# google/layered-scene-inference

Hardware: AMD Instinct MI355X
Metric: rendered views/sec (BxLxHxW splat+warp) (higher is better)
Workload: dtype f32; 1 GPU; cfg3: 4-layer LDI 256x768, batch 32 per GPU (32 total), trg_downsampling 0.5, kitti cameras, compose_layers, smooth disparities; launch=graph, input_sets_rotated=3, parallelism=batch-sharded replicas x1 (no collective)

## Files before the change

include/lsi_hip.h:

```cpp
#ifndef LSI_HIP_H_
#define LSI_HIP_H_

#include <stddef.h>
#include <stdint.h>

#ifdef __cplusplus
extern "C" {
#endif

#define LSI_VERSION 100

#define LSI_OK 0
#define LSI_EINVAL -1
#define LSI_ENULL -2
#define LSI_EWORKSPACE -3
#define LSI_ELAUNCH -4
#define LSI_EUNSUPPORTED -5

#define LSI_COMPOSE 1u
#define LSI_WANT_DISP 2u
#define LSI_HAS_MASK 4u
#define LSI_WS_KEEP 8u
#define LSI_DETERMINISTIC 16u

#define LSI_PACKED_RGBD 32u
#define LSI_GRAD_M 64u

#define LSI_PATH_AUTO 0
#define LSI_PATH_ATOMIC 1
#define LSI_PATH_ROWBAND 2
#define LSI_PATH_STREAM 3

#define LSI_PATH_TILE 4

typedef void* lsi_stream_t;

typedef struct LsiStreamAdapt {
  int32_t state;
  int32_t pending;
  uint32_t seq;
  uint32_t calls;
  uint32_t* ctr_dev;
  volatile uint32_t* ctr_host;
} LsiStreamAdapt;

typedef struct LsiSplatDesc {
  int32_t L, B, H, W, Ht, Wt;
  int64_t tex_sl, tex_sb, tex_sy, tex_sx, tex_sc;
  int64_t disp_sl, disp_sb, disp_sy, disp_sx;
  int64_t mask_sl, mask_sb, mask_sy, mask_sx;
  float trg_downsampling;
  float max_disp;
  float zbuf_scale;
  float bg_wt;
  uint32_t flags;
  int32_t path;
  int32_t tune_rows, tune_threads, tune_window, reserved;
  LsiStreamAdapt* adapt;
} LsiSplatDesc;

int lsi_version(void);

const char* lsi_strerror(int code);

float lsi_bg_weight(double bg_layer_disp, double max_disp, double zbuf_scale);

int lsi_rowband_ok(const LsiSplatDesc* desc, const float* M_host);

int lsi_stream_ok(const LsiSplatDesc* desc, const float* M_host);

size_t lsi_splat_workspace_bytes(const LsiSplatDesc* desc);

int lsi_splat_fwd(const LsiSplatDesc* desc, const float* tex, const float* disp,
                  const float* mask, const float* M, float* out_img,
                  float* out_wts, float* out_disp, void* workspace,
                  size_t workspace_bytes, lsi_stream_t stream);

size_t lsi_splat_bwd_workspace_bytes(const LsiSplatDesc* desc);

int lsi_splat_bwd(const LsiSplatDesc* desc, const float* tex, const float* disp,
                  const float* mask, const float* M, const float* out_img,
                  const float* out_wts, const float* g_img, const float* g_wts,
                  float* g_tex, float* g_disp_in, float* g_mask,
                  void* workspace, size_t workspace_bytes, lsi_stream_t stream);

int lsi_splat_bwd_m(const LsiSplatDesc* desc, const float* tex,
                    const float* disp, const float* mask, const float* M,
                    const float* out_img, const float* out_wts,
                    const float* g_img, const float* g_wts, float* g_tex,
                    float* g_disp_in, float* g_mask, float* g_M, void* workspace,
                    size_t workspace_bytes, lsi_stream_t stream);

size_t lsi_splat_bwd_disp_workspace_bytes(const LsiSplatDesc* desc);

int lsi_splat_bwd_disp(const LsiSplatDesc* desc, const float* tex,
                       const float* disp, const float* mask, const float* M,
                       const float* out_img, const float* out_wts,
                       const float* out_disp, const float* g_img,
                       const float* g_wts, const float* g_disp_out,
                       float* g_tex, float* g_disp_in, float* g_mask,
                       float* g_M, void* workspace, size_t workspace_bytes,
                       lsi_stream_t stream);

int lsi_splat_fwd_both(const LsiSplatDesc* desc, const float* tex,
                       const float* disp, const float* mask, const float* M,
                       float* out_img, float* out_wts, float* out_img_c,
                       float* out_wts_c, void* workspace,
                       size_t workspace_bytes, lsi_stream_t stream);

int lsi_splat_bwd_both(const LsiSplatDesc* desc, const float* tex,
                       const float* disp, const float* mask, const float* M,
                       const float* out_img, const float* out_wts,
                       const float* out_img_c, const float* out_wts_c,
                       const float* g_img, const float* g_wts,
                       const float* g_img_c, const float* g_wts_c, float* g_tex,
                       float* g_disp_in, float* g_mask, void* workspace,
                       size_t workspace_bytes, lsi_stream_t stream);

int lsi_splat_bwd_both_m(const LsiSplatDesc* desc, const float* tex,
                         const float* disp, const float* mask, const float* M,
                         const float* out_img, const float* out_wts,
                         const float* out_img_c, const float* out_wts_c,
                         const float* g_img, const float* g_wts,
                         const float* g_img_c, const float* g_wts_c,
                         float* g_tex, float* g_disp_in, float* g_mask,
                         float* g_M, void* workspace, size_t workspace_bytes,
                         lsi_stream_t stream);

int lsi_project_indices(const LsiSplatDesc* desc, const float* disp,
                        const float* mask, const float* M, int32_t* idx4,
                        float* upd4, lsi_stream_t stream);

int lsi_splat_generic(int32_t B, int32_t Hs, int32_t Ws, int32_t C, int32_t Ht,
                      int32_t Wt, const float* src, const float* coords,
                      float* out, lsi_stream_t stream);

int lsi_splat_generic_bwd(int32_t B, int32_t Hs, int32_t Ws, int32_t C,
                          int32_t Ht, int32_t Wt, const float* src,
                          const float* coords, const float* g_out, float* g_src,
                          float* g_coords, lsi_stream_t stream);

int lsi_projection_matrices(int32_t B, const float* k_s, const float* k_t,
                            const float* rot, const float* t, int32_t inverse,
                            float* M);

int lsi_scatter_add(int32_t B, int64_t P, int64_t N, const int32_t* idx,
                    const float* upd, float* out, lsi_stream_t stream);

int lsi_bilinear_fwd(int32_t B, int32_t Hs, int32_t Ws, int32_t C, int32_t Ht,
                     int32_t Wt, const float* imgs, const float* coords,
                     float* out, lsi_stream_t stream);

int lsi_bilinear_taps(int32_t B, int32_t Hs, int32_t Ws, int32_t C, int32_t Ht,
                      int32_t Wt, const float* imgs, const float* coords,
                      float* taps, float* wts, lsi_stream_t stream);
int lsi_bilinear_taps_bwd(int32_t B, int32_t Hs, int32_t Ws, int32_t C, int32_t Ht,
                          int32_t Wt, const float* coords, const float* g_taps,
                          const float* g_wts, float* g_imgs, float* g_coords,
                          lsi_stream_t stream);

int lsi_bilinear_bwd(int32_t B, int32_t Hs, int32_t Ws, int32_t C, int32_t Ht,
// ... 445 lines not shown
```

layered-scene-inference_amd/csrc/lsi_splat_bwd_stream.hip:

```cpp
#include <hip/hip_runtime.h>
#include <math.h>
#include <stdint.h>
#include <stdlib.h>

#include <type_traits>

#include "../../include/lsi_hip.h"
#include "lsi_common.h"
#include "lsi_splat_internal.h"

#pragma clang fp contract(off)

using namespace lsi;

namespace {

constexpr int BS_WPE = 2;
constexpr int BS_FENCE = 1;
constexpr int BS_T = 512;
constexpr int BS_NW = BS_T / 64;
constexpr int BS_SEG = 256;

struct BSCanvas {
  const float* img;
  const float* wts;
  const float* g_img;
  const float* g_wts;
};

struct BSArgs {
  const float* tex;
  const float* disp;
  const float* M;
  const float* mask;
  float* g_mask;
  int mask_sb, mask_sl, mask_sy;
  BSCanvas ci, cc;
  int vec4;
  float* g_tex;
  float* g_disp;
  int nt;
  int B, H, W, Ht, Wt, L, nseg;
  int tex_sb, tex_sl, tex_sy, disp_sb, disp_sl, disp_sy;
  float s, max_disp, zscale, zA, zB;
  int compose;
  int remap;
  int RS;
  int GR;
  float* gm_part;
  const float2* gd;
};

struct BSIn { float4 d4, t0, t1, t2, mk; };

__device__ __forceinline__ float4 bs_pre(float i0, float i1, float i2, float w,
                                         float g0, float g1, float g2, float gw) {
  const float inv = 1.0f / safe_den(w);
  return make_float4(g0 * inv, g1 * inv, g2 * inv,
                     gw - (g0 * i0 + g1 * i1 + g2 * i2) * inv);
}
__device__ __forceinline__ float4 bs_cell(const BSCanvas& c, size_t o) {
  return bs_pre(c.img[3 * o], c.img[3 * o + 1], c.img[3 * o + 2], c.wts[o],
                c.g_img[3 * o], c.g_img[3 * o + 1], c.g_img[3 * o + 2],
                c.g_wts ? c.g_wts[o] : 0.0f);
}
__device__ __forceinline__ float4 bs_G(const BSArgs& a, size_t oi, size_t oc) {
  float4 g = make_float4(0.f, 0.f, 0.f, 0.f);
  if (a.cc.g_img) g = bs_cell(a.cc, oc);
  if (a.ci.g_img) {
    const float4 h = bs_cell(a.ci, oi);
    g.x += h.x; g.y += h.y; g.z += h.z; g.w += h.w;
  }
  return g;
}
__device__ __forceinline__ void bs_cell4(const BSCanvas& c, size_t o, float4 (&g)[4],
                                         bool add) {
  const float4 ia = *reinterpret_cast<const float4*>(c.img + 3 * o);
  const float4 ib = *reinterpret_cast<const float4*>(c.img + 3 * o + 4);
  const float4 ic = *reinterpret_cast<const float4*>(c.img + 3 * o + 8);
  const float4 w = *reinterpret_cast<const float4*>(c.wts + o);
  const float4 ga = *reinterpret_cast<const float4*>(c.g_img + 3 * o);
  const float4 gb = *reinterpret_cast<const float4*>(c.g_img + 3 * o + 4);
  const float4 gc = *reinterpret_cast<const float4*>(c.g_img + 3 * o + 8);
  float4 gw = make_float4(0.f, 0.f, 0.f, 0.f);
  if (c.g_wts) gw = *reinterpret_cast<const float4*>(c.g_wts + o);
  float4 h[4];
  h[0] = bs_pre(ia.x, ia.y, ia.z, w.x, ga.x, ga.y, ga.z, gw.x);
  h[1] = bs_pre(ia.w, ib.x, ib.y, w.y, ga.w, gb.x, gb.y, gw.y);
  h[2] = bs_pre(ib.z, ib.w, ic.x, w.z, gb.z, gb.w, gc.x, gw.z);
  h[3] = bs_pre(ic.y, ic.z, ic.w, w.w, gc.y, gc.z, gc.w, gw.w);
#pragma unroll
  for (int k = 0; k < 4; ++k) {
    if (add) { g[k].x += h[k].x; g[k].y += h[k].y; g[k].z += h[k].z; g[k].w += h[k].w; }
    else g[k] = h[k];
  }
}

template <bool PACK>
__device__ __forceinline__ void bs_load(BSIn& o, const float* pd, const float* pt) {
  if (PACK) {
    o.d4 = *reinterpret_cast<const float4*>(pt);
    o.t0 = *reinterpret_cast<const float4*>(pt + 4);
    o.t1 = *reinterpret_cast<const float4*>(pt + 8);
    o.t2 = *reinterpret_cast<const float4*>(pt + 12);
  } else {
    o.d4 = *reinterpret_cast<const float4*>(pd);
    o.t0 = *reinterpret_cast<const float4*>(pt);
    o.t1 = *reinterpret_cast<const float4*>(pt + 4);
    o.t2 = *reinterpret_cast<const float4*>(pt + 8);
  }
}

typedef float __attribute__((ext_vector_type(4))) bs_f4v;
typedef const __attribute__((address_space(3))) bs_f4v bs_lds_f4;

template <bool IN_LDS, bool PACK, bool MASK, bool GRAD_M, bool WANT_DISP>
__device__ __forceinline__ void bs_run(const BSArgs& a, const float (&m)[8],
                                       BSIn (&set)[2], const float4* gt,
                                       size_t obi, size_t obc, int b,
                                       int l_lo, int NL, int ys, int nitem,
                                       int glo, int wave, int lane,
                                       float (&acc)[16]) {
  const int Wt = a.Wt, nseg = a.nseg;
  const int half = (Wt + 1) >> 1;
  const float s = a.s;
  const float xmax = (float)Wt - 1.0f, ymax = (float)a.Ht - 1.0f;
  const float inv_md = div_rn(1.0f, a.max_disp);
  const float zs_md = a.zscale * inv_md;
  const float* const g_tex_in = a.tex + (long)b * a.tex_sb + (long)l_lo * a.tex_sl;
  const float* const g_disp_in = a.disp + (long)b * a.disp_sb + (long)l_lo * a.disp_sl;
  const int px_last = a.W - 4;
  const float* const g_mask_in =
      MASK ? a.mask + (long)b * a.mask_sb + (long)l_lo * a.mask_sl : nullptr;
  float* const o_mask =
      MASK ? a.g_mask + ((size_t)l_lo * a.B + b) * ((size_t)a.H * a.W) + 4 * lane : nullptr;
  float* const o_tex = a.g_tex + ((size_t)l_lo * a.B + b) * ((size_t)a.H * a.W) * 3 + 12 * lane;
  float* const o_disp = a.g_disp + ((size_t)l_lo * a.B + b) * ((size_t)a.H * a.W) + 4 * lane;
  const size_t lay_px = (size_t)a.B * a.H * a.W;
  bs_lds_f4* const gt3 = (bs_lds_f4*)gt;

  struct Pos { int r, sg, l; };
  auto advance = [&](Pos& p, int n) {
    p.l += n;
    while (p.l >= NL) { p.l -= NL; ++p.sg; }
    while (p.sg >= nseg) { p.sg -= nseg; ++p.r; }
  };
  auto load_item = [&](BSIn& o, const Pos& p, bool live) {
    const Pos q = live ? p : Pos{0, 0, 0};
    const int px = min(q.sg * BS_SEG + 4 * lane, px_last);
    bs_load<PACK>(o, g_disp_in + (long)q.l * a.disp_sl + (long)(ys + q.r) * a.disp_sy + px,
                  g_tex_in + (long)q.l * a.tex_sl + (long)(ys + q.r) * a.tex_sy + (PACK ? 4 : 3) * px);
    if (MASK)
      o.mk = *reinterpret_cast<const float4*>(
          g_mask_in + (long)q.l * a.mask_sl + (long)(ys + q.r) * a.mask_sy + px);
  };
  auto item = [&](const BSIn& in, const Pos& p) {
    const int y = ys + p.r, sg = p.sg, l = p.l;
    const float py = (float)y + 0.5f;
    const float q1 = mrow(m, 1, 0.5f, py, 0.0f);
    const float Y = q1 * s - 0.5f;
    const Axis ay = splat_axis(Y, ymax);
    const bool yok = finite_f(Y);
    const int r0 = yok ? (int)ay.c0s : glo, r1 = yok ? (int)ay.c1s : glo;
    const float pym01 = py * m[1];
    const float dvn[4] = {in.d4.x, in.d4.y, in.d4.z, in.d4.w};
    const float dvp[4] = {in.d4.w, in.t0.w, in.t1.w, in.t2.w};
    const float txn[12] = {in.t0.x, in.t0.y, in.t0.z, in.t0.w, in.t1.x, in.t1.y,
                           in.t1.z, in.t1.w, in.t2.x, in.t2.y, in.t2.z, in.t2.w};
    const float txp[12] = {in.d4.x, in.d4.y, in.d4.z, in.t0.x, in.t0.y, in.t0.z,
                           in.t1.x, in.t1.y, in.t1.z, in.t2.x, in.t2.y, in.t2.z};
    const float (&dv)[4] = PACK ? dvp : dvn;
    const float (&tx)[12] = PACK ? txp : txn;
    const float mkv[4] = {in.mk.x, in.mk.y, in.mk.z, in.mk.w};
    float ot[12], od[4], om[4];
#pragma unroll
    for (int i = 0; i < 4; ++i) {
      const float d = dv[i];
      const float t0 = tx[3 * i], t1 = tx[3 * i + 1], t2 = tx[3 * i + 2];
      const float px = (float)(sg * BS_SEG + 4 * lane + i) + 0.5f;
      const float q0 = ((px * m[0] + pym01) + m[2]) + d * m[3];
      const float X = q0 * s - 0.5f;
      const bool ok = yok && finite_f(X) && finite_f(d);
      const Axis ax = splat_axis(X, xmax);
      float w0 = clamp_small(ax.w0 * ay.w0), w1 = clamp_small(ax.w1 * ay.w0);
      float w2 = clamp_small(ax.w0 * ay.w1), w3 = clamp_small(ax.w1 * ay.w1);
      if (!ok) { w0 = 0.f; w1 = 0.f; w2 = 0.f; w3 = 0.f; }
      const int c0 = ok ? (int)ax.c0s : 0, c1 = ok ? (int)ax.c1s : 0;
      float4 g0, g1, g2, g3;
      if (IN_LDS) {
        bs_lds_f4* ra = gt3 + (r0 - glo) * Wt;
        bs_lds_f4* rb = gt3 + (r1 - glo) * Wt;
        const int s0 = (c0 >> 1) + (c0 & 1) * half, s1 = (c1 >> 1) + (c1 & 1) * half;
        const bs_f4v v0 = ra[s0], v1 = ra[s1], v2 = rb[s0], v3 = rb[s1];
        g0 = make_float4(v0.x, v0.y, v0.z, v0.w); g1 = make_float4(v1.x, v1.y, v1.z, v1.w);
        g2 = make_float4(v2.x, v2.y, v2.z, v2.w); g3 = make_float4(v3.x, v3.y, v3.z, v3.w);
      } else {
        const size_t ra = (size_t)r0 * Wt, rb = (size_t)r1 * Wt;
        g0 = bs_G(a, obi + ra + c0, obc + ra + c0);
        g1 = bs_G(a, obi + ra + c1, obc + ra + c1);
        g2 = bs_G(a, obi + rb + c0, obc + rb + c0);
        g3 = bs_G(a, obi + rb + c1, obc + rb + c1);
      }
      float gsd = 0.0f;
      if (WANT_DISP) {
        const float2* gdl = a.gd + ((size_t)(l_lo + l) * a.B + b) * ((size_t)a.Ht * Wt);
        const size_t ra = (size_t)r0 * Wt, rb = (size_t)r1 * Wt;
        const float2 e0 = gdl[ra + c0], e1 = gdl[ra + c1];
        const float2 e2 = gdl[rb + c0], e3 = gdl[rb + c1];
        const float dz = ok ? d : 0.0f;
        g0.w = g0.w + (e0.y + dz * e0.x); g1.w = g1.w + (e1.y + dz * e1.x);
        g2.w = g2.w + (e2.y + dz * e2.x); g3.w = g3.w + (e3.y + dz * e3.x);
        gsd = __fmaf_rn(w3, e3.x, __fmaf_rn(w2, e2.x, __fmaf_rn(w1, e1.x, w0 * e0.x)));
      }
      const float xn = d * inv_md;
      const float ez = __builtin_amdgcn_exp2f(
          __fmaf_rn(__builtin_amdgcn_fmed3f(d, 0.0f, a.max_disp), a.zA, a.zB));
      const float zw = xn > 0.0f ? ez : 0.0f;
      const float S0 = __fmaf_rn(t0, g0.x, __fmaf_rn(t1, g0.y, __fmaf_rn(t2, g0.z, g0.w)));
      const float S1 = __fmaf_rn(t0, g1.x, __fmaf_rn(t1, g1.y, __fmaf_rn(t2, g1.z, g1.w)));
      const float S2 = __fmaf_rn(t0, g2.x, __fmaf_rn(t1, g2.y, __fmaf_rn(t2, g2.z, g2.w)));
      const float S3 = __fmaf_rn(t0, g3.x, __fmaf_rn(t1, g3.y, __fmaf_rn(t2, g3.z, g3.w)));
      const float a0 = __fmaf_rn(w3, g3.x, __fmaf_rn(w2, g2.x, __fmaf_rn(w1, g1.x, w0 * g0.x)));
      const float a1 = __fmaf_rn(w3, g3.y, __fmaf_rn(w2, g2.y, __fmaf_rn(w1, g1.y, w0 * g0.y)));
      const float a2 = __fmaf_rn(w3, g3.z, __fmaf_rn(w2, g2.z, __fmaf_rn(w1, g1.z, w0 * g0.z)));
      const float gpw = __fmaf_rn(w3, S3, __fmaf_rn(w2, S2, __fmaf_rn(w1, S1, w0 * S0)));
      const float pw = MASK ? zw * mkv[i] : zw;
      ot[3 * i] = a0 * pw; ot[3 * i + 1] = a1 * pw; ot[3 * i + 2] = a2 * pw;
      if (MASK) om[i] = gpw * zw;
      const float k0 = w0 != 0.0f ? pw * S0 : 0.0f, k1 = w1 != 0.0f ? pw * S1 : 0.0f;
      const float k2 = w2 != 0.0f ? pw * S2 : 0.0f, k3 = w3 != 0.0f ? pw * S3 : 0.0f;
      const float gX = -ax.v0 * (k0 * ay.w0 + k2 * ay.w1) + ax.v1 * (k1 * ay.w0 + k3 * ay.w1);
      const float inr = (xn >= 0.0f && xn <= 1.0f) ? 1.0f : 0.0f;
      float gD = gpw * pw * zs_md * inr;
      if (WANT_DISP) gD += gsd * pw;
      const float gd = (gX * s) * m[3] + gD;
      od[i] = ok ? gd : 0.0f;
      if (GRAD_M && ok && sg * BS_SEG + 4 * lane < a.W) {
        const float gY = -ay.v0 * (k0 * ax.w0 + k1 * ax.w1) +
                         ay.v1 * (k2 * ax.w0 + k3 * ax.w1);
        const float gq0 = gX * s, gq1 = gY * s;
        const float gn = -(gq0 * q0 + gq1 * q1 + gD * d);
        grad_m_add(acc, gq0, gq1, gn, gD, px, py, d);
      }
      if (((i + 1) & ((1 << BS_FENCE) - 1)) == 0 && i < 3) asm volatile("" ::: "memory");
    }
    const size_t po = (size_t)l * lay_px + (size_t)y * a.W + (size_t)sg * BS_SEG;
    if (sg * BS_SEG + 4 * lane < a.W) {
      float* pt = o_tex + 3 * po;
      if (a.nt) {
        store_stream_f4(pt, ot[0], ot[1], ot[2], ot[3]);
        store_stream_f4(pt + 4, ot[4], ot[5], ot[6], ot[7]);
        store_stream_f4(pt + 8, ot[8], ot[9], ot[10], ot[11]);
        store_stream_f4(o_disp + po, od[0], od[1], od[2], od[3]);
        if (MASK) store_stream_f4(o_mask + po, om[0], om[1], om[2], om[3]);
      } else {
        *reinterpret_cast<float4*>(pt) = make_float4(ot[0], ot[1], ot[2], ot[3]);
        *reinterpret_cast<float4*>(pt + 4) = make_float4(ot[4], ot[5], ot[6], ot[7]);
        *reinterpret_cast<float4*>(pt + 8) = make_float4(ot[8], ot[9], ot[10], ot[11]);
        *reinterpret_cast<float4*>(o_disp + po) = make_float4(od[0], od[1], od[2], od[3]);
        if (MASK)
          *reinterpret_cast<float4*>(o_mask + po) = make_float4(om[0], om[1], om[2], om[3]);
      }
    }
  };

  Pos p0{0, 0, 0}, p1{0, 0, 0};
  advance(p0, wave);
  advance(p1, wave + BS_NW);
  for (int it = wave; it < nitem; it += 2 * BS_NW) {
    item(set[0], p0);
    advance(p0, 2 * BS_NW);
    load_item(set[0], p0, it + 2 * BS_NW < nitem);
    if (it + BS_NW < nitem) item(set[1], p1);
    advance(p1, 2 * BS_NW);
    load_item(set[1], p1, it + 3 * BS_NW < nitem);
  }
}

template <bool PACK, bool MASK, bool GRAD_M, bool WANT_DISP>
__global__ __launch_bounds__(BS_T, BS_WPE) void splat_bwd_stream_kernel(BSArgs a) {
  extern __shared__ __attribute__((aligned(16))) unsigned char smem[];
  float4* const gt = reinterpret_cast<float4*>(smem);
  const int tid = threadIdx.x, lane = tid & 63;
  const int wave = __builtin_amdgcn_readfirstlane(tid >> 6);
  int bx = blockIdx.x, by = blockIdx.y, bz = blockIdx.z;
  if (a.remap) {
    const unsigned nbx = gridDim.x, L = gridDim.z;
    const unsigned lin = blockIdx.x + nbx * (blockIdx.y + gridDim.y * blockIdx.z);
    const unsigned xcd = lin & 7u, slot = lin >> 3;
    const unsigned l = slot % L, pair = (slot / L) * 8u + xcd;
    bz = (int)l;
    by = (int)(pair / nbx);
    bx = (int)(pair - (unsigned)by * nbx);
  }
  const int b = by;
  const int ys = bx * a.RS, ye = min(a.H, ys + a.RS);
  const int l_lo = a.compose ? 0 : bz;
  const int NL = a.compose ? a.L : 1;
  const int Wt = a.Wt;
  const int nseg = a.nseg;
  const int nitem = (ye - ys) * nseg * NL;

  BSIn set[2];
  {
    const float* const g_tex_in = a.tex + (long)b * a.tex_sb + (long)l_lo * a.tex_sl;
    const float* const g_disp_in = a.disp + (long)b * a.disp_sb + (long)l_lo * a.disp_sl;
#pragma unroll
    for (int k = 0; k < 2; ++k) {
      const int it = wave + k * BS_NW;
      const int itc = it < nitem ? it : 0;
      const int rs = itc / NL, l = itc - rs * NL;
      const int r = rs / nseg, sg = rs - r * nseg;
      const int px = min(sg * BS_SEG + 4 * lane, a.W - 4);
      bs_load<PACK>(set[k], g_disp_in + (long)l * a.disp_sl + (long)(ys + r) * a.disp_sy + px,
                    g_tex_in + (long)l * a.tex_sl + (long)(ys + r) * a.tex_sy + (PACK ? 4 : 3) * px);
      if (MASK)
        set[k].mk = *reinterpret_cast<const float4*>(
            a.mask + (long)b * a.mask_sb + (long)(l_lo + l) * a.mask_sl +
            (long)(ys + r) * a.mask_sy + px);
    }
  }

  const float* __restrict__ mg = a.M + 16 * b;
  float m[8];
#pragma unroll
  for (int k = 0; k < 8; ++k) m[k] = mg[k];
  const float s = a.s;
  const float ymax = (float)a.Ht - 1.0f;
  auto row_Y = [&](int y) {
    const float py = (float)y + 0.5f;
    return mrow(m, 1, 0.5f, py, 0.0f) * s - 0.5f;
  };
  int glo = 0, ghi = 0;
  {
    const Axis a0 = splat_axis(row_Y(ys), ymax), a1 = splat_axis(row_Y(max(ye - 1, ys)), ymax);
    const float lo = fminf(fminf(a0.c0s, a1.c0s), fminf(a0.c1s, a1.c1s));
    const float hi = fmaxf(fmaxf(a0.c0s, a1.c0s), fmaxf(a0.c1s, a1.c1s));
    glo = finite_f(lo) ? (int)lo : 0;
    ghi = finite_f(hi) ? (int)hi : 0;
  }
  const int grow = ghi - glo + 1;
  const bool in_lds = grow <= a.GR;
  const size_t P = (size_t)a.Ht * Wt;
  const size_t obi = ((size_t)l_lo * a.B + b) * P, obc = (size_t)b * P;
  if (in_lds) {
    const size_t c0 = (size_t)glo * Wt;
    const int n = grow * Wt;
    if (a.vec4) {
      const int half = (Wt + 1) >> 1;
      const float inv_wt = 1.0f / (float)Wt;
      for (int i = 4 * tid; i < n; i += 4 * BS_T) {
        float4 g[4];
#pragma unroll
        for (int k = 0; k < 4; ++k) g[k] = make_float4(0.f, 0.f, 0.f, 0.f);
        if (a.cc.g_img) bs_cell4(a.cc, obc + c0 + i, g, false);
        if (a.ci.g_img) bs_cell4(a.ci, obi + c0 + i, g, a.cc.g_img != nullptr);
        int row = (int)((float)i * inv_wt);
        int c = i - row * Wt;
        if (c >= Wt) { ++row; c -= Wt; }
        if (c < 0) { --row; c += Wt; }
        float4* dst = gt + row * Wt + (c >> 1);
        dst[0] = g[0]; dst[half] = g[1]; dst[1] = g[2]; dst[half + 1] = g[3];
      }
    } else {
      const int half = (Wt + 1) >> 1;
      for (int i = tid; i < n; i += BS_T) {
        const int row = i / Wt, c = i - row * Wt;
        gt[row * Wt + (c >> 1) + (c & 1) * half] = bs_G(a, obi + c0 + i, obc + c0 + i);
      }
    }
  }
  __syncthreads();
  float acc[16];
#pragma unroll
  for (int k = 0; k < 16; ++k) acc[k] = 0.0f;
  if (!GRAD_M && nitem <= 0) return;
  if (nitem > 0) {
    if (in_lds)
      bs_run<true, PACK, MASK, GRAD_M, WANT_DISP>(a, m, set, gt, obi, obc, b, l_lo, NL,
                                                  ys, nitem, glo, wave, lane, acc);
    else
      bs_run<false, PACK, MASK, GRAD_M, WANT_DISP>(a, m, set, gt, obi, obc, b, l_lo, NL,
                                                   ys, nitem, glo, wave, lane, acc);
  }
  if (GRAD_M) {
    __shared__ float red[BS_NW * 16];
    const size_t wg = ((size_t)b * gridDim.z + bz) * gridDim.x + bx;
    grad_m_block_sum<BS_NW>(acc, red, a.gm_part + 16 * wg);
  }
}

}

bool lsi_bwd_stream_applies(const LsiSplatDesc* d, const float* tex,
                            const float* disp, const float* mask,
                            const float* g_tex, const float* g_disp,
                            const float* g_mask) {
  if (const char* e = getenv("LSI_BWD_STREAM"))
    if (e[0] == '0') return false;
  if (d->path != LSI_PATH_STREAM || !(d->tune_window & LSI_STREAM_SIMPLE_BIT))
    return false;
  if (d->flags & LSI_WANT_DISP) return false;
  if (d->flags & LSI_HAS_MASK) {
    if (!mask || !g_mask || (d->flags & LSI_PACKED_RGBD) || d->mask_sx != 1) return false;
    const int64_t ms[] = {d->mask_sl, d->mask_sb, d->mask_sy};
    for (int64_t v : ms)
      if (v < 0 || v > 0x7fffffffLL || v % 4) return false;
    if (!aligned16(mask) || !aligned16(g_mask)) return false;
  }
  if (d->W % 4 != 0 || d->W < 4 || d->L < 1) return false;
  const bool pack = (d->flags & LSI_PACKED_RGBD) != 0;
  if (!pack && (d->tex_sc != 1 || d->tex_sx != 3 || d->disp_sx != 1)) return false;
  const int64_t st[] = {d->tex_sl, d->tex_sb, d->tex_sy, d->disp_sl, d->disp_sb, d->disp_sy};
  for (int64_t v : st)
    if (v < 0 || v > 0x7fffffffLL || v % 4) return false;
  if (!aligned16(tex) || (!pack && !aligned16(disp)) || !aligned16(g_tex) ||
      !aligned16(g_disp))
    return false;
  if ((long)d->B > 65535 || (long)d->L > 65535) return false;
  return true;
}

int lsi_bwd_stream_launch(const LsiSplatDesc* d, const float* tex,
                          const float* disp, const float* mask, const float* M,
                          const LsiBwdCanvas* ci, const LsiBwdCanvas* cc,
                          float* g_tex, float* g_disp, float* g_mask,
                          float* gm_part, int* gm_nper, hipStream_t stream,
                          const float2* gd) {
  BSArgs a;
  a.gm_part = gm_part;
  a.gd = gd;
  a.tex = tex; a.disp = disp; a.M = M; a.g_tex = g_tex; a.g_disp = g_disp;
  {
    static const char* nt_env = getenv("LSI_BWD_NT");
    a.nt = nt_env ? atoi(nt_env) : 0;
  }
  const bool has_mask = (d->flags & LSI_HAS_MASK) != 0;
  a.mask = has_mask ? mask : nullptr; a.g_mask = has_mask ? g_mask : nullptr;
  a.mask_sb = (int)d->mask_sb; a.mask_sl = (int)d->mask_sl; a.mask_sy = (int)d->mask_sy;
  const LsiBwdCanvas none = {nullptr, nullptr, nullptr, nullptr};
  const LsiBwdCanvas& i_ = ci ? *ci : none;
  const LsiBwdCanvas& c_ = cc ? *cc : none;
  a.ci = {i_.img, i_.wts, i_.g_img, i_.g_wts};
  a.cc = {c_.img, c_.wts, c_.g_img, c_.g_wts};
  a.vec4 = d->Wt % 4 == 0;
  for (const BSCanvas* c : {&a.ci, &a.cc})
    if (c->g_img)
      a.vec4 = a.vec4 && aligned16(c->img) && aligned16(c->wts) &&
               aligned16(c->g_img) && aligned16(c->g_wts);
  a.B = d->B; a.H = d->H; a.W = d->W; a.Ht = d->Ht; a.Wt = d->Wt; a.L = d->L;
  a.nseg = (d->W + BS_SEG - 1) / BS_SEG;
  a.tex_sb = (int)d->tex_sb; a.tex_sl = (int)d->tex_sl; a.tex_sy = (int)d->tex_sy;
  a.disp_sb = (int)d->disp_sb; a.disp_sl = (int)d->disp_sl; a.disp_sy = (int)d->disp_sy;
  a.s = d->trg_downsampling; a.max_disp = d->max_disp; a.zscale = d->zbuf_scale;
  const double l2e = 1.4426950408889634;
  a.zA = (float)((double)d->zbuf_scale * l2e / (double)d->max_disp);
  a.zB = (float)(-0.5 * (double)d->zbuf_scale * l2e);
  a.compose = (d->flags & LSI_COMPOSE) ? 1 : 0;
  auto rows_for = [&](int rs) { return (int)ceilf((float)rs * d->trg_downsampling) + 3; };
  auto bytes_for = [&](int rs) { return (size_t)rows_for(rs) * d->Wt * 16; };
  const size_t cap = 156 * 1024;
  int rs = 0;
  if (const char* e = getenv("LSI_BWD_STREAM_ROWS")) rs = atoi(e);
  if (rs <= 0) {
    rs = 8;
    for (int c : {32, 16, 8})
      if (bytes_for(c) <= cap) { rs = c; break; }
    const long nz = a.compose ? 1 : d->L;
    while (rs > 8 && (long)((d->H + rs - 1) / rs) * d->B * nz < 256) rs >>= 1;
  }
  a.RS = rs;
  a.GR = rows_for(rs);
  size_t lds = bytes_for(rs);
  if (lds > cap) { a.GR = 0; lds = 0; }
  const bool pack = (d->flags & LSI_PACKED_RGBD) != 0;
#define BS_FN(P_, M_, G_, D_) ((const void*)splat_bwd_stream_kernel<P_, M_, G_, D_>)
#define BS_PICK(G_, D_)                                                        \
  (pack ? BS_FN(true, false, G_, D_)                                            \
        : (has_mask ? BS_FN(false, true, G_, D_) : BS_FN(false, false, G_, D_)))
  const void* fn = gd ? (gm_part ? BS_PICK(true, true) : BS_PICK(false, true))
                      : (gm_part ? BS_PICK(true, false) : BS_PICK(false, false));
#undef BS_PICK
#undef BS_FN
  if (hipFuncSetAttribute(fn, hipFuncAttributeMaxDynamicSharedMemorySize,
                          (int)(lds > 0 ? lds : 16)) != hipSuccess) {
    (void)hipGetLastError();
    a.GR = 0; lds = 0;
    if (hipFuncSetAttribute(fn, hipFuncAttributeMaxDynamicSharedMemorySize, 16) !=
        hipSuccess)
      return LSI_ELAUNCH;
  }
  const dim3 grid((d->H + rs - 1) / rs, d->B, a.compose ? 1 : d->L);
  if (gm_nper) *gm_nper = (int)(grid.x * grid.z);
  {
    static const char* rm = getenv("LSI_BWD_REMAP");
    const long nwg = (long)grid.x * grid.y * grid.z;
    a.remap = (!a.compose && grid.z > 1 && nwg % (8L * grid.z) == 0 &&
               !(rm && rm[0] == '0')) ? 1 : 0;
  }
  void* kargs[1] = {&a};
  if (hipLaunchKernel(fn, grid, dim3(BS_T), kargs, lds, stream) != hipSuccess)
    return LSI_ELAUNCH;
  return hipGetLastError() == hipSuccess ? LSI_OK : LSI_ELAUNCH;
}
```

layered-scene-inference_amd/lsi/_C.py:

```python
import ctypes
import os

import torch

_PKG = os.path.dirname(os.path.dirname(os.path.abspath(__file__)))
SO_PATH = os.path.join(_PKG, 'liblsi_hip_%s.so' % os.environ['LSI_HIP_LIB'] if
                       os.environ.get('LSI_HIP_LIB') else 'liblsi_hip.so')

LSI_OK = 0
LSI_COMPOSE, LSI_WANT_DISP, LSI_HAS_MASK, LSI_WS_KEEP = 1, 2, 4, 8
LSI_DETERMINISTIC = 16
LSI_PACKED_RGBD = 32
LSI_GRAD_M = 64
LSI_PATH_AUTO, LSI_PATH_ATOMIC, LSI_PATH_ROWBAND, LSI_PATH_STREAM = 0, 1, 2, 3
LSI_PATH_TILE = 4
LSI_SCENE_IMG, LSI_SCENE_DISP, LSI_SCENE_IMG_ROOM, LSI_SCENE_DISP_ROOM = 1, 2, 4, 8
LSI_SCENE_MAX_PLANES = 16
LSI_FC_BN, LSI_FC_X_F32, LSI_FC_OUT_F32 = 1, 2, 4
LSI_IMAGE_MAX_PIXELS = 16843009
LSI_AUG_FLIP = 1
LSI_VIS_SKIP, LSI_VIS_RGB, LSI_VIS_GRAY, LSI_VIS_LUT, LSI_VIS_ABSDIFF = 0, 1, 2, 3, 4
LSI_VIS_MAX_ITEMS = 256
LSI_LIDAR_INVERSE = 1
LSI_DEPTH_SUP_SILOG, LSI_DEPTH_SUP_L1 = 0, 1
# ... 61 lines not shown
      [('reserved', ctypes.c_int32)])


class LsiConvDesc(ctypes.Structure):
  _fields_ = [(n, ctypes.c_int32) for n in (
      'N', 'H', 'W', 'Cin', 'OH', 'OW', 'Cout', 'KH', 'KW', 'stride', 'pad_t', 'pad_l')]


class LsiSceneDesc(ctypes.Structure):
  _fields_ = ([(n, ctypes.c_int32) for n in ('B', 'V', 'P', 'Hs', 'Ws', 'H', 'W',
                                             'n_box', 'soft')] +
              [('min_disp', ctypes.c_float), ('temp', ctypes.c_float),
               ('outputs', ctypes.c_uint32)])


class LsiFcDesc(ctypes.Structure):
  _fields_ = ([(n, ctypes.c_int32) for n in ('M', 'K', 'N', 'groups', 'taps')] +
              [('flags', ctypes.c_uint32), ('w_sn', ctypes.c_int64),
               ('w_sk', ctypes.c_int64), ('tap_off', ctypes.c_int64 * 4),
               ('eps', ctypes.c_float), ('reserved', ctypes.c_int32)])


class LsiPackJob(ctypes.Structure):
  _fields_ = ([('w', ctypes.c_void_p), ('dst', ctypes.c_void_p)] +
              [(n, ctypes.c_int32) for n in ('D0', 'D1', 'khw', 'tr', 'ntaps', 'block0')] +
              [('tap', ctypes.c_int8 * 56)])


class LsiConvIO(ctypes.Structure):
  _fields_ = ([(n, ctypes.c_void_p) for n in ('x', 'x2', 'packed', 'out', 'out2',
                                              'bn_workspace', 'workspace')] +
              [('workspace_bytes', ctypes.c_size_t), ('c1', ctypes.c_int32),
               ('groups', ctypes.c_int32)])


class LsiImageDesc(ctypes.Structure):
  _fields_ = ([('offset', ctypes.c_int64)] +
              [(n, ctypes.c_int32) for n in ('H', 'W', 'C', 'reserved')])


class LsiAugmentDesc(ctypes.Structure):
  _fields_ = ([('offset', ctypes.c_int64)] +
              [(n, ctypes.c_int32) for n in ('H', 'W', 'C')] +
              [('flags', ctypes.c_uint32)] +
              [(n, ctypes.c_int32) for n in ('y0', 'x0', 'ch', 'cw', 'table',
                                             'reserved')] +
              [('gain', ctypes.c_float * 3), ('reserved2', ctypes.c_int32)])


class LsiVisSheet(ctypes.Structure):
  _fields_ = ([(n, ctypes.c_int32) for n in ('rows', 'cols', 'cell_h', 'cell_w',
                                             'gutter', 'n_items')] +
              [('bg', ctypes.c_uint8 * 3), ('nan', ctypes.c_uint8 * 3),
               ('reserved', ctypes.c_uint8 * 2)])


class LsiScanDesc(ctypes.Structure):
  _fields_ = [('first', ctypes.c_int64), ('n', ctypes.c_int32),
              ('reserved', ctypes.c_int32)]


class LsiVisItem(ctypes.Structure):
  _fields_ = ([('src', ctypes.c_void_p), ('ref', ctypes.c_void_p)] +
              [(n, ctypes.c_int64) for n in ('s_y', 's_x', 's_c', 'r_y', 'r_x', 'r_c')] +
              [(n, ctypes.c_int32) for n in ('kind', 'H', 'W', 'C', 'zoom', 'reserved')] +
              [('lo', ctypes.c_float), ('inv', ctypes.c_float)])


_I32, _I64, _VP, _SZ = ctypes.c_int32, ctypes.c_int64, ctypes.c_void_p, ctypes.c_size_t
_DP = ctypes.POINTER(LsiSplatDesc)
_LP = ctypes.POINTER(LsiLossDesc)
_CP = ctypes.POINTER(LsiConvDesc)
_F32 = ctypes.c_float
SIGNATURES = {
    'lsi_version': (ctypes.c_int, []),
    'lsi_strerror': (ctypes.c_char_p, [ctypes.c_int]),
    'lsi_bg_weight': (ctypes.c_float, [ctypes.c_double] * 3),
    'lsi_rowband_ok': (ctypes.c_int, [_DP, _VP]),
    'lsi_stream_ok': (ctypes.c_int, [_DP, _VP]),
    'lsi_splat_workspace_bytes': (_SZ, [_DP]),
    'lsi_stream_adapt_state': (ctypes.c_int, [ctypes.POINTER(LsiStreamAdapt)]),
    'lsi_splat_fwd': (ctypes.c_int, [_DP] + [_VP] * 8 + [_SZ, _VP]),
    'lsi_splat_bwd_workspace_bytes': (_SZ, [_DP]),
    'lsi_splat_bwd': (ctypes.c_int, [_DP] + [_VP] * 12 + [_SZ, _VP]),
    'lsi_splat_bwd_m': (ctypes.c_int, [_DP] + [_VP] * 13 + [_SZ, _VP]),
    'lsi_splat_bwd_disp_workspace_bytes': (_SZ, [_DP]),
    'lsi_splat_bwd_disp': (ctypes.c_int, [_DP] + [_VP] * 15 + [_SZ, _VP]),
    'lsi_splat_fwd_both': (ctypes.c_int, [_DP] + [_VP] * 9 + [_SZ, _VP]),
    'lsi_splat_bwd_both': (ctypes.c_int, [_DP] + [_VP] * 16 + [_SZ, _VP]),
    'lsi_splat_bwd_both_m': (ctypes.c_int, [_DP] + [_VP] * 17 + [_SZ, _VP]),
    'lsi_project_indices': (ctypes.c_int, [_DP] + [_VP] * 6),
    'lsi_splat_generic': (ctypes.c_int, [_I32] * 6 + [_VP] * 4),
    'lsi_splat_generic_bwd': (ctypes.c_int, [_I32] * 6 + [_VP] * 6),
    'lsi_scatter_add': (ctypes.c_int, [_I32, _I64, _I64] + [_VP] * 4),
    'lsi_bilinear_fwd': (ctypes.c_int, [_I32] * 6 + [_VP] * 4),
    'lsi_conv3x3_pred_bwd_workspace_bytes': (_SZ, [_I32] * 3),
    'lsi_conv3x3_wgrad_workspace_bytes': (_SZ, [_I32] * 5),
    'lsi_conv3x3_wgrad': (ctypes.c_int, [_I32] * 5 + [_VP] * 4 + [_SZ, _VP]),
    'lsi_conv3x3_pred_bwd': (ctypes.c_int, [_I32] * 4 + [_VP] * 7 + [_SZ, _VP]),
    'lsi_conv3x3_c32_fwd': (ctypes.c_int, [_I32] * 5 + [_VP] * 3 + [_F32, _VP, _VP]),
    'lsi_projection_matrices': (ctypes.c_int, [_I32] + [_VP] * 4 + [_I32, _VP]),
    'lsi_bilinear_taps': (ctypes.c_int, [_I32] * 6 + [_VP] * 5),
    'lsi_bilinear_bwd': (ctypes.c_int, [_I32] * 6 + [_VP] * 6),
    'lsi_bilinear_taps_bwd': (ctypes.c_int, [_I32] * 6 + [_VP] * 5 + [_VP]),
    'lsi_loss_workspace_bytes': (_SZ, []),
    'lsi_zbuf_comp_loss_fwd': (ctypes.c_int, [_LP] + [_VP] * 6 + [_SZ, _VP]),
    'lsi_zbuf_comp_loss_bwd': (ctypes.c_int, [_LP] + [_VP] * 9),
    'lsi_disp_reg_loss_fwd': (ctypes.c_int, [_I32] * 4 + [_I64] * 4 + [_VP] * 3 +
                              [_SZ, _VP]),
    'lsi_disp_reg_loss_bwd': (ctypes.c_int, [_I32] * 4 + [_I64] * 4 + [_VP] * 4),
    'lsi_view_synth_loss_fwd': (ctypes.c_int, [_I32] * 8 + [_VP] * 2 + [_I64] * 4 +
                                [_VP] * 2 + [_SZ, _VP]),
    'lsi_view_synth_loss_bwd': (ctypes.c_int, [_I32] * 8 + [_VP] * 2 + [_I64] * 4 +
                                [_VP] * 3),
    'lsi_ssim_window': (ctypes.c_int, [_I32, _F32, _VP]),
    'lsi_ssim_loss_fwd': (ctypes.c_int, [ctypes.POINTER(LsiSsimDesc)] + [_VP] * 4 +
                          [_SZ, _VP]),
    'lsi_ssim_loss_bwd': (ctypes.c_int, [ctypes.POINTER(LsiSsimDesc)] + [_VP] * 5),
    'lsi_eval_ssim': (ctypes.c_int, [ctypes.POINTER(LsiSsimDesc)] + [_VP] * 4 +
                      [_SZ, _VP]),
    'lsi_edge_smooth_workspace_bytes': (_SZ, [ctypes.POINTER(LsiEdgeSmoothDesc)]),
    'lsi_edge_smooth_loss_fwd': (ctypes.c_int, [ctypes.POINTER(LsiEdgeSmoothDesc)] +
                                 [_VP] * 5 + [_SZ, _VP]),
    'lsi_edge_smooth_loss_bwd': (ctypes.c_int, [ctypes.POINTER(LsiEdgeSmoothDesc)] +
                                 [_VP] * 6),
    'lsi_depth_sup_workspace_bytes': (_SZ, [ctypes.POINTER(LsiDepthSupDesc)]),
    'lsi_depth_sup_loss_fwd': (ctypes.c_int, [ctypes.POINTER(LsiDepthSupDesc)] +
                               [_VP] * 6 + [_SZ, _VP]),
    'lsi_depth_sup_loss_bwd': (ctypes.c_int, [ctypes.POINTER(LsiDepthSupDesc)] +
                               [_VP] * 7),
    'lsi_compose_fwd': (ctypes.c_int, [_I32, _I64, _I32] + [_VP] * 3 +
                        [_I32, _F32, _F32, _VP, _VP]),
    'lsi_compose_depth_fwd': (ctypes.c_int, [_I32, _I64] + [_VP] * 2 +
                              [_I32, _F32, _F32, _F32, _VP, _VP]),
    'lsi_compose_bwd': (ctypes.c_int, [_I32, _I64, _I32] + [_VP] * 3 +
                        [_I32, _F32, _F32] + [_VP] * 5),
    'lsi_compose_depth_bwd': (ctypes.c_int, [_I32, _I64] + [_VP] * 2 +
                              [_I32, _F32, _F32, _F32] + [_VP] * 3),
    'lsi_eval_workspace_bytes': (_SZ, []),
    'lsi_eval_view_metrics': (ctypes.c_int, [_I32] * 8 + [_VP] * 3 + [_I64] * 4 +
                              [_VP] * 3 + [ctypes.c_uint32, _F32] + [_VP] * 2 +
                              [_SZ, _VP]),
    'lsi_eval_layer_metrics': (ctypes.c_int, ([_LP] + [_VP] * 6) * 2 + [_VP] * 2 +
                               [_SZ, _VP]),
    'lsi_eval_depth_workspace_bytes': (_SZ, [_I32] * 4),
    'lsi_eval_depth_metrics': (ctypes.c_int, [_I32] * 3 + [_VP] * 4 + [_I32] * 4 +
                               [_F32] * 3 + [ctypes.c_uint32] + [_VP] * 3 + [_SZ, _VP]),
    'lsi_disocclusion_mask': (ctypes.c_int, [_I32] * 5 + [_VP] * 3 + [_F32, _VP, _VP]),
    'lsi_render_planes': (ctypes.c_int, [ctypes.POINTER(LsiSceneDesc)] + [_VP] * 8),
    'lsi_render_planes_bwd_workspace_bytes': (_SZ, [ctypes.POINTER(LsiSceneDesc)]),
    'lsi_render_planes_bwd': (ctypes.c_int, [ctypes.POINTER(LsiSceneDesc)] +
                              [_VP] * 9 + [_SZ, _VP]),
    'lsi_conv2d_supported': (ctypes.c_int, [_CP]),
    'lsi_conv2d_packed_bytes': (_SZ, [_CP]),
    'lsi_conv2d_pack': (ctypes.c_int, [_CP, _I32, _VP, _VP, _SZ, _VP]),
    'lsi_conv2d_pack_job': (ctypes.c_int, [_CP, _I32, _VP, _VP, _SZ,
                                           ctypes.POINTER(LsiPackJob), _c_i]),
    'lsi_conv2d_pack_many': (ctypes.c_int, [_VP, _I32, _I32, _VP]),
    'lsi_conv2d_fwd': (ctypes.c_int, [_CP] + [_VP] * 4),
    'lsi_conv2d_bwd_data': (ctypes.c_int, [_CP] + [_VP] * 4),
    'lsi_conv2d_fwd_bnstats': (ctypes.c_int, [_CP] + [_VP] * 4 + [_I32, _VP]),
    'lsi_conv2d_bwd_data_bnstats': (ctypes.c_int, [_CP] + [_VP] * 4 + [_I32, _VP]),
    'lsi_conv2d_fwd_cat': (ctypes.c_int, [_CP, _VP, _VP, _I32, _VP, _VP, _VP, _I32, _VP]),
    'lsi_conv2d_bwd_data_cat': (ctypes.c_int, [_CP, _VP, _VP, _VP, _VP, _I32, _VP]),
    'lsi_conv2d_wgrad_cat': (ctypes.c_int, [_CP, _VP, _VP, _I32, _VP, _VP, _I32, _VP, _SZ, _VP]),
    'lsi_conv2d_workspace_bytes': (_SZ, [_CP, _I32]),
# ... 115 lines not shown
```

Before: 389,800 views/s.

## Stage bwd-stream texture gradients through LDS slabs and allow 768-thread blocks

The backward stream splat kernel now writes each wave's per-lane 12-float texture gradient into a per-wave LDS slab and reads it back so each lane stores contiguous float4 lines. This is meant to produce fully coalesced streaming stores instead of 48-byte strided per-lane writes. A planner also selects 768-thread blocks for lean configurations (no mask, grad-M or disp) when the canvas plus slabs fit in the LDS cap, and exposes the plan through a new API. The costs are extra LDS traffic and a waitcnt per item, plus more LDS per block, which may reduce occupancy.

```diff
diff --git a/include/lsi_hip.h b/include/lsi_hip.h
--- a/include/lsi_hip.h
+++ b/include/lsi_hip.h
@@ -77,6 +77,9 @@
                   size_t workspace_bytes, lsi_stream_t stream);
 
 size_t lsi_splat_bwd_workspace_bytes(const LsiSplatDesc* desc);
+
+int lsi_splat_bwd_stream_plan(const LsiSplatDesc* desc, int rows, int store,
+                              int threads, int32_t* out);
 
 int lsi_splat_bwd(const LsiSplatDesc* desc, const float* tex, const float* disp,
                   const float* mask, const float* M, const float* out_img,
diff --git a/layered-scene-inference_amd/csrc/lsi_splat_bwd_stream.hip b/layered-scene-inference_amd/csrc/lsi_splat_bwd_stream.hip
--- a/layered-scene-inference_amd/csrc/lsi_splat_bwd_stream.hip
+++ b/layered-scene-inference_amd/csrc/lsi_splat_bwd_stream.hip
@@ -15,11 +15,14 @@
 
 namespace {
 
-constexpr int BS_WPE = 2;
 constexpr int BS_FENCE = 1;
-constexpr int BS_T = 512;
-constexpr int BS_NW = BS_T / 64;
+constexpr int BS_T_MIN = 512, BS_T_MAX = 768;
 constexpr int BS_SEG = 256;
+constexpr int BS_ST_PLAIN = 0;
+constexpr int BS_ST_NT = 1;
+constexpr int BS_ST_LINES = 2;
+constexpr int BS_SLAB = BS_SEG * 12;
+constexpr size_t BS_LDS_CAP = 156 * 1024;
 
 struct BSCanvas {
   const float* img;
@@ -40,6 +43,7 @@
   float* g_tex;
   float* g_disp;
   int nt;
+  int slab_off;
   int B, H, W, Ht, Wt, L, nseg;
   int tex_sb, tex_sl, tex_sy, disp_sb, disp_sl, disp_sy;
   float s, max_disp, zscale, zA, zB;
@@ -114,9 +118,10 @@
 typedef float __attribute__((ext_vector_type(4))) bs_f4v;
 typedef const __attribute__((address_space(3))) bs_f4v bs_lds_f4;
 
-template <bool IN_LDS, bool PACK, bool MASK, bool GRAD_M, bool WANT_DISP>
+template <int NW, bool LINES, bool IN_LDS, bool PACK, bool MASK, bool GRAD_M, bool WANT_DISP>
 __device__ __forceinline__ void bs_run(const BSArgs& a, const float (&m)[8],
                                        BSIn (&set)[2], const float4* gt,
+                                       float4* slab,
                                        size_t obi, size_t obc, int b,
                                        int l_lo, int NL, int ys, int nitem,
                                        int glo, int wave, int lane,
@@ -134,7 +139,8 @@
       MASK ? a.mask + (long)b * a.mask_sb + (long)l_lo * a.mask_sl : nullptr;
   float* const o_mask =
       MASK ? a.g_mask + ((size_t)l_lo * a.B + b) * ((size_t)a.H * a.W) + 4 * lane : nullptr;
-  float* const o_tex = a.g_tex + ((size_t)l_lo * a.B + b) * ((size_t)a.H * a.W) * 3 + 12 * lane;
+  float* const o_tex_seg = a.g_tex + ((size_t)l_lo * a.B + b) * ((size_t)a.H * a.W) * 3;
+  float* const o_tex = o_tex_seg + 12 * lane;
   float* const o_disp = a.g_disp + ((size_t)l_lo * a.B + b) * ((size_t)a.H * a.W) + 4 * lane;
   const size_t lay_px = (size_t)a.B * a.H * a.W;
   bs_lds_f4* const gt3 = (bs_lds_f4*)gt;
@@ -245,9 +251,28 @@
       if (((i + 1) & ((1 << BS_FENCE) - 1)) == 0 && i < 3) asm volatile("" ::: "memory");
     }
     const size_t po = (size_t)l * lay_px + (size_t)y * a.W + (size_t)sg * BS_SEG;
-    if (sg * BS_SEG + 4 * lane < a.W) {
+    if (LINES) {
+      if (sg * BS_SEG + 4 * lane < a.W) {
+        store_stream_f4(o_disp + po, od[0], od[1], od[2], od[3]);
+        if (MASK) store_stream_f4(o_mask + po, om[0], om[1], om[2], om[3]);
+      }
+      LSI_COMPILER_FENCE();
+      slab[3 * lane] = make_float4(ot[0], ot[1], ot[2], ot[3]);
+      slab[3 * lane + 1] = make_float4(ot[4], ot[5], ot[6], ot[7]);
+      slab[3 * lane + 2] = make_float4(ot[8], ot[9], ot[10], ot[11]);
+      asm volatile("s_waitcnt lgkmcnt(0)" ::: "memory");
+      const int nch = 3 * (min(BS_SEG, a.W - sg * BS_SEG) >> 2);
+      float* const seg = o_tex_seg + 3 * po;
+#pragma unroll
+      for (int j = 0; j < 3; ++j) {
+        const int c = 64 * j + lane;
+        const float4 v = slab[c];
+        if (c < nch) store_stream_f4(seg + 4 * c, v.x, v.y, v.z, v.w);
+      }
+      LSI_COMPILER_FENCE();
+    } else if (sg * BS_SEG + 4 * lane < a.W) {
       float* pt = o_tex + 3 * po;
-      if (a.nt) {
+      if (a.nt == BS_ST_NT) {
         store_stream_f4(pt, ot[0], ot[1], ot[2], ot[3]);
         store_stream_f4(pt + 4, ot[4], ot[5], ot[6], ot[7]);
         store_stream_f4(pt + 8, ot[8], ot[9], ot[10], ot[11]);
@@ -266,19 +291,20 @@
 
   Pos p0{0, 0, 0}, p1{0, 0, 0};
   advance(p0, wave);
-  advance(p1, wave + BS_NW);
-  for (int it = wave; it < nitem; it += 2 * BS_NW) {
+  advance(p1, wave + NW);
+  for (int it = wave; it < nitem; it += 2 * NW) {
     item(set[0], p0);
-    advance(p0, 2 * BS_NW);
-    load_item(set[0], p0, it + 2 * BS_NW < nitem);
-    if (it + BS_NW < nitem) item(set[1], p1);
-    advance(p1, 2 * BS_NW);
-    load_item(set[1], p1, it + 3 * BS_NW < nitem);
-  }
-}
-
-template <bool PACK, bool MASK, bool GRAD_M, bool WANT_DISP>
-__global__ __launch_bounds__(BS_T, BS_WPE) void splat_bwd_stream_kernel(BSArgs a) {
+    advance(p0, 2 * NW);
+    load_item(set[0], p0, it + 2 * NW < nitem);
+    if (it + NW < nitem) item(set[1], p1);
+    advance(p1, 2 * NW);
+    load_item(set[1], p1, it + 3 * NW < nitem);
+  }
+}
+
+template <int BS_T, bool LINES, bool PACK, bool MASK, bool GRAD_M, bool WANT_DISP>
+__global__ __launch_bounds__(BS_T, BS_T / 256) void splat_bwd_stream_kernel(BSArgs a) {
+  constexpr int BS_NW = BS_T / 64;
   extern __shared__ __attribute__((aligned(16))) unsigned char smem[];
   float4* const gt = reinterpret_cast<float4*>(smem);
   const int tid = threadIdx.x, lane = tid & 63;
@@ -375,13 +401,14 @@
 #pragma unroll
   for (int k = 0; k < 16; ++k) acc[k] = 0.0f;
   if (!GRAD_M && nitem <= 0) return;
+  float4* const slab = reinterpret_cast<float4*>(smem + a.slab_off + wave * BS_SLAB);
   if (nitem > 0) {
     if (in_lds)
-      bs_run<true, PACK, MASK, GRAD_M, WANT_DISP>(a, m, set, gt, obi, obc, b, l_lo, NL,
-                                                  ys, nitem, glo, wave, lane, acc);
+      bs_run<BS_NW, LINES, true, PACK, MASK, GRAD_M, WANT_DISP>(
+          a, m, set, gt, slab, obi, obc, b, l_lo, NL, ys, nitem, glo, wave, lane, acc);
     else
-      bs_run<false, PACK, MASK, GRAD_M, WANT_DISP>(a, m, set, gt, obi, obc, b, l_lo, NL,
-                                                   ys, nitem, glo, wave, lane, acc);
+      bs_run<BS_NW, LINES, false, PACK, MASK, GRAD_M, WANT_DISP>(
+          a, m, set, gt, slab, obi, obc, b, l_lo, NL, ys, nitem, glo, wave, lane, acc);
   }
   if (GRAD_M) {
     __shared__ float red[BS_NW * 16];
@@ -421,6 +448,56 @@
   return true;
 }
 
+namespace {
+struct BSPlan {
+  int rows, canvas_rows, threads, store;
+  size_t canvas_bytes, slab_bytes;
+};
+BSPlan bs_plan(const LsiSplatDesc* d, int rows, int store, int threads, bool lean) {
+  BSPlan p;
+  auto rows_for = [&](int rs) { return (int)ceilf((float)rs * d->trg_downsampling) + 3; };
+  auto bytes_for = [&](int rs) { return (size_t)rows_for(rs) * d->Wt * 16; };
+  int rs = rows;
+  if (rs <= 0) {
+    rs = 8;
+    for (int c : {32, 16, 8})
+      if (bytes_for(c) <= BS_LDS_CAP) { rs = c; break; }
+    const long nz = (d->flags & LSI_COMPOSE) ? 1 : d->L;
+    while (rs > 8 && (long)((d->H + rs - 1) / rs) * d->B * nz < 256) rs >>= 1;
+  }
+  p.rows = rs;
+  p.canvas_rows = rows_for(rs);
+  p.canvas_bytes = bytes_for(rs);
+  if (p.canvas_bytes > BS_LDS_CAP) { p.canvas_rows = 0; p.canvas_bytes = 0; }
+  p.store = store >= BS_ST_PLAIN && store <= BS_ST_LINES ? store : BS_ST_LINES;
+  auto slabs_for = [&](int t) { return (size_t)(t / 64) * BS_SLAB; };
+  auto fits = [&](int t) { return p.canvas_bytes + slabs_for(t) <= BS_LDS_CAP; };
+  if (threads == BS_T_MIN || threads == BS_T_MAX) p.threads = threads;
+  else p.threads = p.store == BS_ST_LINES && fits(BS_T_MIN) && !fits(BS_T_MAX) ? BS_T_MIN
+                                                                                : BS_T_MAX;
+  if (!lean) p.threads = BS_T_MIN;
+  p.slab_bytes = 0;
+  if (p.store == BS_ST_LINES) {
+    if (fits(p.threads)) p.slab_bytes = slabs_for(p.threads);
+    else p.store = BS_ST_PLAIN;
+  }
+  return p;
+}
+bool bs_lean(const LsiSplatDesc* d) {
+  return !(d->flags & (LSI_HAS_MASK | LSI_GRAD_M | LSI_WANT_DISP));
+}
+}
+
+int lsi_splat_bwd_stream_plan(const LsiSplatDesc* d, int rows, int store, int threads,
+                              int32_t* out) {
+  if (!d || !out) return LSI_ENULL;
+  if (d->Wt < 1 || d->H < 1 || d->B < 1 || d->L < 1) return LSI_EINVAL;
+  const BSPlan p = bs_plan(d, rows, store, threads, bs_lean(d));
+  out[0] = p.rows; out[1] = p.canvas_rows; out[2] = p.threads; out[3] = p.store;
+  out[4] = (int32_t)p.canvas_bytes; out[5] = (int32_t)p.slab_bytes;
+  return LSI_OK;
+}
+
 int lsi_bwd_stream_launch(const LsiSplatDesc* d, const float* tex,
                           const float* disp, const float* mask, const float* M,
                           const LsiBwdCanvas* ci, const LsiBwdCanvas* cc,
@@ -431,10 +508,10 @@
   a.gm_part = gm_part;
   a.gd = gd;
   a.tex = tex; a.disp = disp; a.M = M; a.g_tex = g_tex; a.g_disp = g_disp;
-  {
-    static const char* nt_env = getenv("LSI_BWD_NT");
-    a.nt = nt_env ? atoi(nt_env) : 0;
-  }
+  int want_store = -1, want_threads = 0, want_rows = 0;
+  if (const char* e = getenv("LSI_BWD_NT")) want_store = atoi(e);
+  if (const char* e = getenv("LSI_BWD_STREAM_THREADS")) want_threads = atoi(e);
+  if (const char* e = getenv("LSI_BWD_STREAM_ROWS")) want_rows = atoi(e);
   const bool has_mask = (d->flags & LSI_HAS_MASK) != 0;
   a.mask = has_mask ? mask : nullptr; a.g_mask = has_mask ? g_mask : nullptr;
   a.mask_sb = (int)d->mask_sb; a.mask_sl = (int)d->mask_sl; a.mask_sy = (int)d->mask_sy;
@@ -457,35 +534,39 @@
   a.zA = (float)((double)d->zbuf_scale * l2e / (double)d->max_disp);
   a.zB = (float)(-0.5 * (double)d->zbuf_scale * l2e);
   a.compose = (d->flags & LSI_COMPOSE) ? 1 : 0;
-  auto rows_for = [&](int rs) { return (int)ceilf((float)rs * d->trg_downsampling) + 3; };
-  auto bytes_for = [&](int rs) { return (size_t)rows_for(rs) * d->Wt * 16; };
-  const size_t cap = 156 * 1024;
-  int rs = 0;
-  if (const char* e = getenv("LSI_BWD_STREAM_ROWS")) rs = atoi(e);
-  if (rs <= 0) {
-    rs = 8;
-    for (int c : {32, 16, 8})
-      if (bytes_for(c) <= cap) { rs = c; break; }
-    const long nz = a.compose ? 1 : d->L;
-    while (rs > 8 && (long)((d->H + rs - 1) / rs) * d->B * nz < 256) rs >>= 1;
-  }
+  const bool lean = !has_mask && !gm_part && !gd;
+  const BSPlan plan = bs_plan(d, want_rows, want_store, want_threads, lean);
+  const int rs = plan.rows;
   a.RS = rs;
-  a.GR = rows_for(rs);
-  size_t lds = bytes_for(rs);
-  if (lds > cap) { a.GR = 0; lds = 0; }
+  a.GR = plan.canvas_rows;
+  a.nt = plan.store;
+  a.slab_off = (int)plan.canvas_bytes;
+  size_t lds = plan.canvas_bytes + plan.slab_bytes;
   const bool pack = (d->flags & LSI_PACKED_RGBD) != 0;
-#define BS_FN(P_, M_, G_, D_) ((const void*)splat_bwd_stream_kernel<P_, M_, G_, D_>)
+  auto pick = [&](bool lines) -> const void* {
+#define BS_FN(T_, P_, M_, G_, D_)                                               \
+  (lines ? (const void*)splat_bwd_stream_kernel<T_, true, P_, M_, G_, D_>       \
+         : (const void*)splat_bwd_stream_kernel<T_, false, P_, M_, G_, D_>)
 #define BS_PICK(G_, D_)                                                        \
-  (pack ? BS_FN(true, false, G_, D_)                                            \
-        : (has_mask ? BS_FN(false, true, G_, D_) : BS_FN(false, false, G_, D_)))
-  const void* fn = gd ? (gm_part ? BS_PICK(true, true) : BS_PICK(false, true))
-                      : (gm_part ? BS_PICK(true, false) : BS_PICK(false, false));
+  (pack ? BS_FN(BS_T_MIN, true, false, G_, D_)                                  \
+        : (has_mask ? BS_FN(BS_T_MIN, false, true, G_, D_)                      \
+                    : BS_FN(BS_T_MIN, false, false, G_, D_)))
+    if (plan.threads == BS_T_MAX)
+      return pack ? BS_FN(BS_T_MAX, true, false, false, false)
+                  : BS_FN(BS_T_MAX, false, false, false, false);
+    return gd ? (gm_part ? BS_PICK(true, true) : BS_PICK(false, true))
+              : (gm_part ? BS_PICK(true, false) : BS_PICK(false, false));
 #undef BS_PICK
 #undef BS_FN
+  };
+  const void* fn = pick(a.nt == BS_ST_LINES);
   if (hipFuncSetAttribute(fn, hipFuncAttributeMaxDynamicSharedMemorySize,
                           (int)(lds > 0 ? lds : 16)) != hipSuccess) {
     (void)hipGetLastError();
     a.GR = 0; lds = 0;
+    a.slab_off = 0;
+    if (a.nt == BS_ST_LINES) a.nt = BS_ST_PLAIN;
+    fn = pick(false);
     if (hipFuncSetAttribute(fn, hipFuncAttributeMaxDynamicSharedMemorySize, 16) !=
         hipSuccess)
       return LSI_ELAUNCH;
@@ -499,7 +580,7 @@
                !(rm && rm[0] == '0')) ? 1 : 0;
   }
   void* kargs[1] = {&a};
-  if (hipLaunchKernel(fn, grid, dim3(BS_T), kargs, lds, stream) != hipSuccess)
+  if (hipLaunchKernel(fn, grid, dim3(plan.threads), kargs, lds, stream) != hipSuccess)
     return LSI_ELAUNCH;
   return hipGetLastError() == hipSuccess ? LSI_OK : LSI_ELAUNCH;
 }
diff --git a/layered-scene-inference_amd/lsi/_C.py b/layered-scene-inference_amd/lsi/_C.py
--- a/layered-scene-inference_amd/lsi/_C.py
+++ b/layered-scene-inference_amd/lsi/_C.py
@@ -167,6 +167,7 @@
     'lsi_stream_adapt_state': (ctypes.c_int, [ctypes.POINTER(LsiStreamAdapt)]),
     'lsi_splat_fwd': (ctypes.c_int, [_DP] + [_VP] * 8 + [_SZ, _VP]),
     'lsi_splat_bwd_workspace_bytes': (_SZ, [_DP]),
+    'lsi_splat_bwd_stream_plan': (ctypes.c_int, [_DP] + [ctypes.c_int] * 3 + [_c_i]),
     'lsi_splat_bwd': (ctypes.c_int, [_DP] + [_VP] * 12 + [_SZ, _VP]),
     'lsi_splat_bwd_m': (ctypes.c_int, [_DP] + [_VP] * 13 + [_SZ, _VP]),
     'lsi_splat_bwd_disp_workspace_bytes': (_SZ, [_DP]),
```

Result: no change. 390,300 views/s, median of 4 (+0.1%).
